# hegdepashupati/zero-inflated-gp

Hardware: AMD Instinct MI355X
Metric: elbo_steps_per_sec (higher is better)
Workload: dtype f64; 1 GPU; dense zero-inflated GP ELBO step (value+gradient), N=1000000 rows per GPU, D=3, M=1024 per latent, full batch; rows_this_rank=1000000, rows_total=1000000, M=1024, D=3, chunk_rows=32768, parallelism=row-shard x1, 1 all-reduce/step

## Files before the change

zero-inflated-gp_amd/csrc/zigp_ctx.h:

```cpp
#pragma once
#include <hip/hip_runtime.h>
#include <stdint.h>
#include <stdio.h>
#include <string.h>
#include <string>
#include <vector>
#include <map>
#include <memory>
#include "../../include/zigp.h"
#include "../../include/zigp_diag.h"
#include "zigp_gemm.h"

namespace zigp {

struct DevBuf {
  double* p = nullptr;
  size_t cap = 0;
  bool owned = true;
  DevBuf() = default;
  DevBuf(const DevBuf&) = delete;
  DevBuf& operator=(const DevBuf&) = delete;
  DevBuf(DevBuf&& o) noexcept : p(o.p), cap(o.cap), owned(o.owned) { o.p = nullptr; o.cap = 0; o.owned = true; }
  DevBuf& operator=(DevBuf&& o) noexcept {
    if (this != &o) { release(); p = o.p; cap = o.cap; owned = o.owned; o.p = nullptr; o.cap = 0; o.owned = true; }
    return *this;
  }
  ~DevBuf() { release(); }
  int ensure(size_t n) {
    if (!owned) { p = nullptr; cap = 0; owned = true; }
    if (n <= cap) return 0;
    if (p) (void)hipFree(p);
    p = nullptr; cap = 0;
    hipError_t e = hipMalloc((void**)&p, n * sizeof(double));
    if (e != hipSuccess) return -1;
    cap = n;
    return 0;
  }
  void alias(double* q, size_t n) { release(); p = q; cap = n; owned = false; }
  void release() { if (p && owned) (void)hipFree(p); p = nullptr; cap = 0; owned = true; }
};

enum ProfClass { PC_GEMM_A1 = 0, PC_GEMM_A2 = 1, PC_GEMM_H = 2, PC_GEMM_J = 3, PC_SYR2K = 4, PC_KUF = 5, PC_POINT = 6, PC_RED = 7, PC_MXM = 8, PC_OTHER = 9 };

struct TileList {
  GemmTile* d = nullptr;
  int n = 0;
  int per = 1;
};
struct HipFree { void operator()(void* q) const { (void)hipFree(q); } };
struct CachedTiles {
  std::unique_ptr<GemmTile, HipFree> d;
  int n = 0, per = 1;
  TileList view() const { return TileList{d.get(), n, per}; }
};

struct Latent {
  int M = 0, Mp = 0;
  DevBuf Z, ell, u, s, s2;
  double zc[64] = {0};
  bool kg_exact = false;
  DevBuf Zs;
  double var = 1.0;
  DevBuf Kuu, L, W;
  DevBuf K, A1, Jp;
  DevBuf Kd;
  DevBuf Wp, a1gm;
  DevBuf Wt;
  DevBuf P, Qt, Rt;
  bool P_ready = false;
  DevBuf part;
  DevBuf gm, gv;
  DevBuf du, dsq, krow;
  DevBuf xm, mom, ks0;
  DevBuf dLpart;
  DevBuf T1, T2, T3, G;
  DevBuf sk;
  DevBuf vec;
  DevBuf wh;
  DevBuf Lraw, Lq, lqssq, dLq;
};

struct KronState;
struct KfState;

struct PinnedArena {
  struct Block { char* p; size_t cap, used; };
  std::vector<Block> blocks;
  PinnedArena() = default;
  PinnedArena(const PinnedArena&) = delete;
  PinnedArena& operator=(const PinnedArena&) = delete;
  ~PinnedArena() { for (auto& b : blocks) (void)hipHostFree(b.p); }
  void reset() { for (auto& b : blocks) b.used = 0; }
  void* alloc(size_t bytes) {
    bytes = (bytes + 63) & ~(size_t)63;
    for (auto& b : blocks)
      if (b.cap - b.used >= bytes) { void* r = b.p + b.used; b.used += bytes; return r; }
    Block nb; nb.cap = bytes > ((size_t)1 << 20) ? bytes : ((size_t)1 << 20); nb.used = bytes; nb.p = nullptr;
    if (hipHostMalloc((void**)&nb.p, nb.cap, hipHostMallocDefault) != hipSuccess) return nullptr;
    blocks.push_back(nb);
    return nb.p;
  }
};

struct CtxHandles {
  hipStream_t stream = nullptr;
  hipStream_t stream_main = nullptr, stream2 = nullptr;
  hipStream_t stream3 = nullptr;
  hipEvent_t ev_fork = nullptr, ev_join = nullptr;
  hipEvent_t ev_prep_fork = nullptr, ev_prep = nullptr;
  int* d_info = nullptr;
  struct PendingEv { hipEvent_t a, b; int cls; };
  std::vector<PendingEv> pending;
  std::vector<hipEvent_t> ev_pool;
  CtxHandles() = default;
  CtxHandles(const CtxHandles&) = delete;
  CtxHandles& operator=(const CtxHandles&) = delete;
  ~CtxHandles() {
    if (d_info) (void)hipFree(d_info);
    for (auto& e : pending) { (void)hipEventDestroy(e.a); (void)hipEventDestroy(e.b); }
    for (auto e : ev_pool) (void)hipEventDestroy(e);
    for (hipEvent_t e : {ev_fork, ev_join, ev_prep_fork, ev_prep})
      if (e) (void)hipEventDestroy(e);
    for (hipStream_t s : {stream3, stream2, stream_main})
      if (s) (void)hipStreamDestroy(s);
  }
};

}

struct zigp_ctx : zigp::CtxHandles {
  ~zigp_ctx();
  int device = 0;
  std::string err;
  int info = 0;
  int64_t fit_steps_applied = 0;
  int64_t chunk = 32768;
  bool chunk_auto = true;
  const double* dX = nullptr; const double* dY = nullptr;
  zigp::DevBuf ownX, ownY;
  int64_t N = 0; int D = 0;
  const double* fullX = nullptr; const double* fullY = nullptr; int64_t fullN = 0;
  zigp::DevBuf selX, selY, selIdx;
  zigp::DevBuf fitX, fitY, fitIdx, fit;
  int64_t dense_fit_steps_applied = 0;
  zigp::Latent lat[2];
  zigp::DevBuf pw_part;
  bool fwd_kuf_side = true;
  bool trmm_tail = true;
  int overlap = 1;
  bool mean_on = false;
  bool whiten = false;
  int kern[2] = {0, 0};
  bool q_full = false;
  double mean_a[8] = {0}, mean_b = 0.0, mean_da[8] = {0}, mean_db = 0.0;
  zigp::DevBuf out9;
  zigp::DevBuf scratch, scratch2;
  zigp::PinnedArena pinned;
  std::unique_ptr<zigp::KronState> kron;
  std::unique_ptr<zigp::KfState> kronf;
  bool kron_panels = false;
  int kron_range_tiles = 1024;
  std::map<std::string, zigp::CachedTiles> tiles;
  void* comm = nullptr; int comm_rank = 0, comm_nranks = 1; int64_t comm_calls = 0;
  double comm_timeout_s = 120.0;
  zigp::DevBuf packed;
  zigp::DevBuf parm;
  double pivot_rtol = 8.0;
  bool prof_on = false;
  int prof_every = 8;
  bool prof_skip = false;
  int64_t prof_total[ZIGP_NCLASS] = {0};
  double prof_ms[ZIGP_NCLASS] = {0};
  int64_t prof_n[ZIGP_NCLASS] = {0};
  double prof_flops[ZIGP_NCLASS] = {0};
};

namespace zigp {

#define ZIGP_HIP(ctx, expr)                                                              \
  do {                                                                                   \
    hipError_t _e = (expr);                                                              \
    if (_e != hipSuccess) {                                                              \
      char _b[512];                                                                      \
      snprintf(_b, sizeof(_b), "HIP error '%s' at %s:%d (%s)", hipGetErrorString(_e), __FILE__, __LINE__, #expr); \
      (ctx)->err = _b;                                                                   \
      return ZIGP_EHIP;                                                                  \
    }                                                                                    \
  } while (0)

#define ZIGP_TRY(expr)            \
  do {                            \
    int _rc = (expr);             \
    if (_rc != 0) return _rc;     \
  } while (0)

#define ZIGP_ENSURE(ctx, buf, n)                                        \
  do {                                                                  \
    if ((buf).ensure((size_t)(n)) != 0) {                               \
      (ctx)->err = "hipMalloc failed for " #buf;                        \
      return ZIGP_EHIP;                                                 \
    }                                                                   \
  } while (0)

inline int fail_arg(zigp_ctx* c, const char* msg) { c->err = msg; return ZIGP_EARG; }
// ... 55 lines not shown
```

zero-inflated-gp_amd/csrc/zigp_dense.hip:

```cpp
#include "zigp_ctx.h"
#include "zigp_kernels.h"
#include "zigp_host.h"
#include "zigp_comm.h"
#include <algorithm>
#include <cmath>
#include <functional>

using namespace zigp;

static_assert(WIDE_MAXD == ZIGP_MAX_D, "the wide kernels' hyperparameter structs hold ZIGP_MAX_D entries");
#define ZIGP_STR2(x) #x
#define ZIGP_STR(x) ZIGP_STR2(x)
#define ZIGP_MAX_D_STR ZIGP_STR(ZIGP_MAX_D)

namespace {

enum class Param : int { Diag = 0, White = 1, WhiteFull = 2 };
constexpr bool is_white(Param p) { return p != Param::Diag; }
constexpr bool is_full(Param p) { return p == Param::WhiteFull; }
static_assert((int)Param::Diag == ZIGP_FIT_DIAG && (int)Param::White == ZIGP_FIT_WHITE && (int)Param::WhiteFull == ZIGP_FIT_WHITE_FULL,
              "Param values are the ZIGP_FIT_* modes of include/zigp.h");
Param param_of(const zigp_ctx* c) { return !c->whiten ? Param::Diag : c->q_full ? Param::WhiteFull : Param::White; }

struct HostLatent {
// ... 204 lines not shown
int latent_chunk_kuf_matern(zigp_ctx* c, Latent& lt, const double* dX, int64_t Nrows, int64_t n0, int64_t Nc, int D, const double* ell_host, int kind,
                            bool with_kd) {
  if (D < 1 || D > MAXD || !ell_host) return fail_arg(c, "a Matern Kuf panel needs 1 <= D <= 8 and host lengthscales");
  if (with_kd && lt.Kd.cap < (size_t)lt.Mp * Nc) return fail_arg(c, "a Matern gradient step's K' panel was not sized for this chunk");
  const KufHyp kh = make_kuf_hyp(ell_host, lt.var, D);
  ProfScope ps(c, PC_KUF);
  const dim3 grid((unsigned)(Nc / 512), lt.Mp / 16), block(256);
#define ZIGP_KUF_M(DD, KK, GG) \
  hipLaunchKernelGGL((k_kuf_build_matern<DD, KK, GG>), grid, block, 0, c->stream, dX, Nrows, n0, lt.Zs.p, lt.M, kh, lt.K.p, GG ? lt.Kd.p : nullptr, Nc)
#define ZIGP_KUF_MD(DD)                                                                    \
  case DD:                                                                                 \
    if (kind == ZIGP_KERN_MATERN32) { if (with_kd) ZIGP_KUF_M(DD, KERN_M32, true); else ZIGP_KUF_M(DD, KERN_M32, false); } \
    else { if (with_kd) ZIGP_KUF_M(DD, KERN_M52, true); else ZIGP_KUF_M(DD, KERN_M52, false); }                            \
    break;
  switch (D) { ZIGP_KUF_MD(1) ZIGP_KUF_MD(2) ZIGP_KUF_MD(3) ZIGP_KUF_MD(4) ZIGP_KUF_MD(5) ZIGP_KUF_MD(6) ZIGP_KUF_MD(7) ZIGP_KUF_MD(8) }
#undef ZIGP_KUF_MD
#undef ZIGP_KUF_M
  ZIGP_HIP(c, hipGetLastError());
  return 0;
}
int latent_chunk_kuf(zigp_ctx* c, Latent& lt, const double* dX, int64_t Nrows, int64_t n0, int64_t Nc, int D, const double* ell_host,
                     const double* R = nullptr, int kind = ZIGP_KERN_RBF, bool with_kd = false) {
  if (is_matern(kind)) return latent_chunk_kuf_matern(c, lt, dX, Nrows, n0, Nc, D, ell_host, kind, with_kd);
  const int Mp = lt.Mp;
  const KufHyp kh = (R || D > MAXD) ? KufHyp() : make_kuf_hyp(ell_host, lt.var, D);
  ProfScope ps(c, PC_KUF);
  const dim3 grid((unsigned)(Nc / 512), Mp / 16), block(256);
#define ZIGP_KUF(DD)                                                                                                                   \
  case DD:                                                                                                                             \
    if (R) hipLaunchKernelGGL((k_kuf_build<DD, LatHypDev>), grid, block, 0, c->stream, dX, Nrows, n0, lt.Zs.p, lt.M, LatHypDev{R, DD}, lt.K.p, Nc); \
    else hipLaunchKernelGGL((k_kuf_build<DD, KufHyp>), grid, block, 0, c->stream, dX, Nrows, n0, lt.Zs.p, lt.M, kh, lt.K.p, Nc);               \
    break;
  switch (D) {
    ZIGP_KUF(1) ZIGP_KUF(2) ZIGP_KUF(3) ZIGP_KUF(4) ZIGP_KUF(5) ZIGP_KUF(6) ZIGP_KUF(7) ZIGP_KUF(8)
    default:
      if (D < 1 || D > WIDE_MAXD || R) return fail_arg(c, "D out of range");
      hipLaunchKernelGGL(k_kuf_build_wide, grid, block, 0, c->stream, dX, Nrows, n0, lt.Zs.p, lt.M, D, make_kuf_hyp_wide(ell_host, lt.var, D), lt.K.p, Nc);
      break;
  }
#undef ZIGP_KUF
  ZIGP_HIP(c, hipGetLastError());
  return 0;
}

struct ChunkPlan {
  int64_t Nc = 0;
  bool paired = false;
  TrmmTail tail = {{0, 0}, {64, 64}};
  struct Lat { TileSpec a1_spec, a2j_spec, syr_spec, mom_spec; TileList a1, a2j, syr, mom; double fl = 0.0; } lat[2];
};
ChunkPlan chunk_plan(const int (&M)[2], int64_t Nc, Param par, bool need_grad, bool tail_on, bool wide) {
  ChunkPlan pl;
  const int nbm[2] = {ceil_div(M[0], BM), ceil_div(M[1], BM)}, nbn = (int)(Nc / BN);
  pl.Nc = Nc;
  pl.paired = trmm_paired_pays(nbn * ((nbm[0] + 1) / 2 + (nbm[1] + 1) / 2));
  if (pl.paired && tail_on)
    pl.tail = trmm_tail_plan((nbn + 7) / 8 * 8 * ((nbm[0] + 1) / 2), nbm[0], (nbn + 7) / 8 * 8 * ((nbm[1] + 1) / 2), nbm[1]);
  for (int h = 0; h < 2; ++h) {
    ChunkPlan::Lat& L = pl.lat[h];
    auto tri = [&](bool lower) { return trmm_tiles(lower, nbm[h], nbn, pl.paired, pl.tail.units[h], pl.tail.bins[h]); };
    auto full_product = [&] { return full_xcd_tiles(nbm[h], nbn, nbm[h] * (BM / BK)); };
    L.a1_spec = tri(true);
    switch (par) {
      case Param::Diag: L.a2j_spec = need_grad ? full_product() : tri(false); break;
      case Param::White: if (need_grad) L.a2j_spec = tri(false); break;
      case Param::WhiteFull: L.a2j_spec = need_grad ? full_product() : tri(false); break;
    }
    if (need_grad) L.syr_spec = syr2k_tiles(nbm[h], (int)(Nc / BK), syr_plan(nbm[h]));
    if (need_grad && wide) L.mom_spec = kgmom_tiles(nbm[h], Nc);
    L.fl = (double)M[h] * M[h] * (double)Nc;
  }
  return pl;
}
int upload_plan(zigp_ctx* c, ChunkPlan& pl) {
  for (ChunkPlan::Lat& L : pl.lat) {
    ZIGP_TRY(get_tiles(c, L.a1_spec, L.a1));
    if (L.a2j_spec.build) ZIGP_TRY(get_tiles(c, L.a2j_spec, L.a2j));
    if (L.syr_spec.build) ZIGP_TRY(get_tiles(c, L.syr_spec, L.syr));
    if (L.mom_spec.build) ZIGP_TRY(get_tiles(c, L.mom_spec, L.mom));
  }
  return 0;
}

int chunk_forward(zigp_ctx* c, const ChunkPlan& pl, Param par, bool need_grad, const std::function<int()>& after_a1 = nullptr) {
  const int64_t Nc = pl.Nc;
  struct Set { TileList t1, t2; double fl; GemmArgs a1, a2j; EpiStoreColsum e1; EpiColsum e2; EpiStorePanelKColsum ej; } q[3] = {};
  for (int h = 0; h < 2; ++h) {
    Latent& lt = c->lat[h];
    const int Mp = lt.Mp, np = Mp / 32;
    q[h].t1 = pl.lat[h].a1; q[h].t2 = pl.lat[h].a2j; q[h].fl = pl.lat[h].fl;
    q[h].a1 = mk_args(lt.Wt.p, Mp, lt.K.p, Nc, lt.A1.p, Nc);
    q[h].e1 = EpiStoreColsum{is_full(par) ? lt.wh.p + Mp : lt.vec.p, nullptr, lt.part.p, lt.part.p + (size_t)np * Nc};
    if (need_grad) {
      q[h].a2j = mk_args(lt.Rt.p, Mp, lt.A1.p, Nc, lt.Jp.p, Nc);
      q[h].ej = EpiStorePanelKColsum{lt.K.p, lt.part.p + (size_t)2 * np * Nc};
    } else {
      q[h].a2j = mk_args(is_full(par) ? lt.Lq.p : lt.W.p, Mp, lt.A1.p, Nc, nullptr, Nc);
      q[h].e2 = EpiColsum{nullptr, is_full(par) ? nullptr : lt.s2.p, nullptr, lt.part.p + (size_t)2 * np * Nc};
    }
  }
  const int groups = pl.paired ? 1 : 2;
  for (int gi = 0; gi < groups; ++gi) {
    const Set& x = q[gi];
    const Set& y = q[pl.paired ? 1 : 2];
    {
      ProfScope ps(c, PC_GEMM_A1, x.fl + y.fl);
      ZIGP_TRY((run_gemm<LAY_MNCONTIG, LAY_MNCONTIG, false, TRI_A_LOWER>(c, x.t1, x.a1, x.e1, y.t1, y.a1, y.e1)));
    }
    if (gi == groups - 1 && after_a1) ZIGP_TRY(after_a1());
    if (need_grad) {
      ProfScope ps(c, PC_GEMM_J, 2.0 * (x.fl + y.fl));
      ZIGP_TRY((run_gemm<LAY_MNCONTIG, LAY_MNCONTIG, false>(c, x.t2, x.a2j, x.ej, y.t2, y.a2j, y.ej)));
    } else {
      ProfScope ps(c, PC_GEMM_A2, x.fl + y.fl);
      ZIGP_TRY((run_gemm<LAY_MNCONTIG, LAY_MNCONTIG, false, TRI_A_UPPER>(c, x.t2, x.a2j, x.e2, y.t2, y.a2j, y.e2)));
    }
  }
  return 0;
}

int chunk_forward_white(zigp_ctx* c, const ChunkPlan& pl, bool need_grad, bool part_j, const std::function<int()>& after_a = nullptr) {
  const int64_t Nc = pl.Nc;
  struct Set { TileList t; double fl; GemmArgs g; EpiStoreColsum es; EpiColsum ec; } q[3] = {};
  for (int h = 0; h < 2; ++h) {
    Latent& lt = c->lat[h];
    const int Mp = lt.Mp, np = Mp / 32;
    double* p0 = lt.part.p; double* p2 = lt.part.p + (size_t)2 * np * Nc;
    q[h].fl = pl.lat[h].fl;
    if (part_j) { q[h].t = pl.lat[h].a2j; q[h].g = mk_args(lt.Wp.p, Mp, lt.A1.p, Nc, lt.Jp.p, Nc); continue; }
    q[h].t = pl.lat[h].a1;
    q[h].g = mk_args(lt.Wt.p, Mp, lt.K.p, Nc, need_grad ? lt.A1.p : nullptr, Nc);
    q[h].es = EpiStoreColsum{lt.wh.p + Mp, lt.wh.p, p0, p2};
    q[h].ec = EpiColsum{lt.wh.p + Mp, lt.wh.p, p0, p2};
  }
  const int groups = pl.paired ? 1 : 2;
  for (int gi = 0; gi < groups; ++gi) {
    const Set& x = q[gi];
    const Set& y = q[pl.paired ? 1 : 2];
    if (part_j) {
      ProfScope ps(c, PC_GEMM_J, x.fl + y.fl);
      ZIGP_TRY((run_gemm<LAY_MNCONTIG, LAY_MNCONTIG, false, TRI_A_UPPER>(c, x.t, x.g, EpiStore(), y.t, y.g, EpiStore())));
      continue;
    }
    {
      ProfScope ps(c, PC_GEMM_A1, x.fl + y.fl);
      if (need_grad) ZIGP_TRY((run_gemm<LAY_MNCONTIG, LAY_MNCONTIG, false, TRI_A_LOWER>(c, x.t, x.g, x.es, y.t, y.g, y.es)));
      else ZIGP_TRY((run_gemm<LAY_MNCONTIG, LAY_MNCONTIG, false, TRI_A_LOWER>(c, x.t, x.g, x.ec, y.t, y.g, y.ec)));
    }
    if (gi == groups - 1 && after_a) ZIGP_TRY(after_a());
  }
  return 0;
}

int latent_chunk_kgrad_wide(zigp_ctx* c, Latent& lt, const double* dX, int64_t Nrows, int64_t n0, int64_t Nc, int D, const TileList& mom) {
  const int Mp = lt.Mp, S = kgmom_slices(Mp / BM, Nc);
  if (mom.n != S * (Mp / BM)) return fail_arg(c, "wide Kuf gradient: the moments product's tile list was not planned for this chunk shape");
  KgCentreWide ctr;
  for (int d = 0; d < WIDE_MAXD; ++d) ctr.c[d] = lt.zc[d];
  hipLaunchKernelGGL(k_kgrad_wide_prep, dim3(Mp / KG_ROWS, KG_SPLIT), dim3(256), 0, c->stream, lt.Jp.p, lt.K.p, lt.vec.p + Mp, lt.gm.p, lt.gv.p, dX, Nrows,
                     n0, lt.M, Mp, D, Nc, (int64_t)Mp * (2 + 2 * D), ctr, lt.krow.p, lt.ks0.p, lt.xm.p);
  ZIGP_HIP(c, hipGetLastError());
  GemmArgs g = mk_args(lt.Jp.p, Nc, lt.xm.p, WIDE_MOM_COLS, lt.mom.p, WIDE_MOM_COLS);
  g.slice_stride = (int64_t)Mp * WIDE_MOM_COLS;
  ZIGP_TRY((run_gemm<LAY_KCONTIG, LAY_MNCONTIG, false>(c, mom, g, EpiStore())));
  hipLaunchKernelGGL(k_kgrad_wide_finish, dim3(Mp / 4), dim3(256), 0, c->stream, lt.mom.p, S, lt.ks0.p, lt.Z.p, lt.M, Mp, D, ctr, lt.krow.p);
  ZIGP_HIP(c, hipGetLastError());
  return 0;
}
int ensure_kgrad_wide(zigp_ctx* c, Latent& lt, int64_t Nc) {
  const int Mp = lt.Mp;
  ZIGP_ENSURE(c, lt.xm, (size_t)Nc * WIDE_MOM_COLS);
  ZIGP_ENSURE(c, lt.mom, (size_t)kgmom_slices(Mp / BM, Nc) * Mp * WIDE_MOM_COLS);
  ZIGP_ENSURE(c, lt.ks0, (size_t)KG_SPLIT * Mp);
  return 0;
}

int latent_chunk_kgrad_matern(zigp_ctx* c, Latent& lt, const double* dX, int64_t Nrows, int64_t n0, int64_t Nc, int D) {
  const int Mp = lt.Mp;
  if (D < 1 || D > MAXD) return fail_arg(c, "a Matern Kuf gradient needs 1 <= D <= 8");
  if (lt.Kd.cap < (size_t)Mp * Nc) return fail_arg(c, "a Matern gradient step's K' panel was not sized for this chunk");
  ProfScope ps(c, PC_RED);
  const dim3 gk((unsigned)ceil_div(lt.M, KG_ROWS), KG_SPLIT), bk(256);
  const int64_t slab = (int64_t)Mp * (2 + 2 * D);
#define ZIGP_KGRAD_M(DD)                                                                                                                         \
  case DD:                                                                                                                                       \
    hipLaunchKernelGGL((k_kgrad_matern<DD>), gk, bk, 0, c->stream, lt.Jp.p, lt.K.p, lt.Kd.p, lt.vec.p + Mp, lt.gm.p, lt.gv.p, dX, Nrows, n0, lt.Z.p, \
                       lt.M, Nc, slab, lt.krow.p);                                                                                               \
    break;
  switch (D) { ZIGP_KGRAD_M(1) ZIGP_KGRAD_M(2) ZIGP_KGRAD_M(3) ZIGP_KGRAD_M(4) ZIGP_KGRAD_M(5) ZIGP_KGRAD_M(6) ZIGP_KGRAD_M(7) ZIGP_KGRAD_M(8) }
#undef ZIGP_KGRAD_M
  ZIGP_HIP(c, hipGetLastError());
  return 0;
// ... 160 lines not shown
    std::string who;
    if (matern_latent(c, who))
      return fail_arg(c, ("a " + who + " (zigp_set_kernel) and D = " + std::to_string(p->D) + ": the Matern kernels cover D in [1, 8] (the wide kernels are RBF only)").c_str());
  }
  if (p->D > MAXD && c->mean_on)
    for (int d = 0; d < MAXD; ++d)
      if (c->mean_a[d] != 0.0) return fail_arg(c, "a Linear mean function is set and D > 8: Linear covers D in [1, 8] (Zero and Constant work at every D)");
  if (!p->Zf || !p->Zg || !p->u_fm || !p->u_gm || !p->u_fs_sqrt || !p->u_gs_sqrt || !p->ell_f || !p->ell_g)
    return fail_arg(c, "NULL pointer in params");
  if (!(p->var_f > 0) || !(p->var_g > 0) || !(p->noise > 0)) return fail_arg(c, "variances must be positive");
  for (int d = 0; d < p->D; ++d)
    if (!(p->ell_f[d] > 0) || !(p->ell_g[d] > 0)) return fail_arg(c, "lengthscales must be positive");
  if (c->q_full) {
    if (!c->whiten) return fail_arg(c, "zigp_set_q_full is on while whitening is off: the full-covariance q(u) exists for the whitened model only (zigp_set_whiten)");
    for (int m = 0; m < p->Mf; ++m)
      if (!(p->u_fs_sqrt[(size_t)m * p->Mf + m] != 0)) return fail_arg(c, "u_fs_sqrt has a zero (or NaN) diagonal entry (full q_sqrt, zigp_set_q_full)");
    for (int m = 0; m < p->Mg; ++m)
      if (!(p->u_gs_sqrt[(size_t)m * p->Mg + m] != 0)) return fail_arg(c, "u_gs_sqrt has a zero (or NaN) diagonal entry (full q_sqrt, zigp_set_q_full)");
    return 0;
  }
  for (int m = 0; m < p->Mf; ++m)
    if (!(p->u_fs_sqrt[m] > 0)) return fail_arg(c, "u_fs_sqrt must be positive (diagonal q_sqrt, transforms.positive)");
  for (int m = 0; m < p->Mg; ++m)
    if (!(p->u_gs_sqrt[m] > 0)) return fail_arg(c, "u_gs_sqrt must be positive (diagonal q_sqrt, transforms.positive)");
  return 0;
}

struct DenseCall {
  const zigp_params* p; const double* dX; const double* dY; int64_t Nrows; int D;
  double jitter, scale, g_offset; int64_t row_begin, row_end; int include_kl; bool predict; double* d_out9;
  bool need_grad, has_rows;
  Param par = Param::Diag;
  bool dlq_as_triangle = false;
  HostLatent hl[2]; const double* ell_h[2];
  int64_t Nc = 0;
  ChunkPlan plan[2];
  int pw_blocks = 0;
  int* hinfo = nullptr;
  bool prep_side = false;
  const double* d_hyp = nullptr; int* d_info2 = nullptr;
  const double* hyp_rec(int h) const { return d_hyp ? d_hyp + h * DH_LAT : nullptr; }
};

int dense_prepare_buffers(zigp_ctx* c, DenseCall& k);
int64_t dense_first_chunk_rows(const DenseCall& k) { return std::min<int64_t>(k.Nc, round_up(k.row_end - k.row_begin, 1024)); }
int dense_mxm_forward(zigp_ctx* c, DenseCall& k) {
  if (k.d_hyp) ZIGP_HIP(c, hipMemsetAsync(k.d_info2, 0, 2 * sizeof(int), c->stream));
  else {
    ZIGP_TRY(begin_staged_call(c));
    ZIGP_HIP(c, hipMemsetAsync(c->d_info, 0, sizeof(int), c->stream));
    ZIGP_TRY(latents_upload(c, k.hl, k.D, k.par));
  }
  k.prep_side = c->overlap == 1 && !c->prof_on;
  if (k.prep_side) {
    ZIGP_TRY(fork_side(c, c->ev_prep_fork, c->stream3));
    OnStream on(c, c->stream3);
    ZIGP_TRY(dense_prepare_buffers(c, k));
    if (k.has_rows)
      for (int h = 0; h < 2; ++h)
        ZIGP_TRY(latent_chunk_kuf(c, c->lat[h], k.dX, k.Nrows, k.row_begin, dense_first_chunk_rows(k), k.D, k.ell_h[h], k.hyp_rec(h), k.hl[h].kind,
                                  k.need_grad));
    ZIGP_HIP(c, hipEventRecord(c->ev_prep, c->stream3));
  }
  {
    ProfScope ps(c, PC_MXM);
    ZIGP_TRY(fork_side(c, c->ev_fork, c->stream2));
    ZIGP_TRY(latents_forward(c, k.hl, k.D, k.jitter, k.par, true, k.need_grad, k.d_hyp, k.d_info2));
    ZIGP_TRY(join_side(c, c->ev_join, c->stream2));
  }
  return k.d_hyp ? 0 : request_info(c, &k.hinfo);
}

int64_t auto_chunk_for(bool chunk_auto, int64_t chunk_set, int64_t Mp) {
  if (!chunk_auto) return chunk_set;
  return std::min<int64_t>(131072, std::max<int64_t>(32768, round_up(32768 * 1024 / std::max<int64_t>(Mp, 128), 1024)));
}
int64_t chunk_rows_for(bool chunk_auto, int64_t chunk_set, int64_t Mp, int64_t span) {
  int64_t chunk = auto_chunk_for(chunk_auto, chunk_set, Mp);
  if (chunk_auto && span > 0 && span <= 131072 && 4 * 2 * 8 * Mp * round_up(span, 1024) <= ((int64_t)9 << 30)) chunk = 131072;
  if (span <= 0) return 1024;
  const int64_t nchunks = (span + chunk - 1) / chunk;
  return std::max<int64_t>(1024, round_up((span + nchunks - 1) / nchunks, 1024));
}
int dense_prepare_buffers(zigp_ctx* c, DenseCall& k) {
  const int64_t Nc = k.Nc;
  const int D = k.D;
  k.pw_blocks = (int)(Nc / PW_PTS);
  ZIGP_ENSURE(c, c->pw_part, (size_t)k.pw_blocks * PW_ACC);
  ZeroRanges zr;
  zr.count = 0;
  static_assert(1 + 2 * 4 <= ZERO_RANGES_MAX, "one launch zeroes every small accumulator of a call");
  auto zero = [&](double* ptr, int64_t n) { zr.p[zr.count] = ptr; zr.n[zr.count] = n; ++zr.count; };
  zero(c->pw_part.p, (int64_t)k.pw_blocks * PW_ACC);
  for (int h = 0; h < 2; ++h) {
    Latent& lt = c->lat[h];
    const int Mp = lt.Mp;
    ZIGP_ENSURE(c, lt.gm, Nc); ZIGP_ENSURE(c, lt.gv, Nc);
    if (k.has_rows) {
      ZIGP_ENSURE(c, lt.K, (size_t)Mp * Nc);
      if (k.par != Param::White || k.need_grad) ZIGP_ENSURE(c, lt.A1, (size_t)Mp * Nc);
      ZIGP_ENSURE(c, lt.part, (size_t)3 * (Mp / 32) * Nc);
      if (k.need_grad) ZIGP_ENSURE(c, lt.Jp, (size_t)Mp * Nc);
      if (k.need_grad && is_matern(k.hl[h].kind)) ZIGP_ENSURE(c, lt.Kd, (size_t)Mp * Nc);
      if (k.need_grad && D > MAXD && !lt.kg_exact) ZIGP_TRY(ensure_kgrad_wide(c, lt, Nc));
    }
    if (k.need_grad) {
      ZIGP_ENSURE(c, lt.du, Mp); ZIGP_ENSURE(c, lt.dsq, Mp); ZIGP_ENSURE(c, lt.krow, (size_t)KG_SPLIT * Mp * (2 + 2 * D));
      const int S = syr_plan(Mp / BM).planes();
      ZIGP_ENSURE(c, lt.dLpart, (size_t)S * Mp * Mp);
      ZIGP_ENSURE(c, lt.a1gm, Mp);
      zero(lt.a1gm.p, Mp); zero(lt.du.p, Mp); zero(lt.dsq.p, Mp); zero(lt.krow.p, (int64_t)KG_SPLIT * Mp * (2 + 2 * D));
      if (k.has_rows) ZIGP_HIP(c, hipMemsetAsync(lt.dLpart.p, 0, sizeof(double) * S * Mp * Mp, c->stream));
    }
  }
  hipLaunchKernelGGL(k_zero_ranges, dim3(64), dim3(256), 0, c->stream, zr);
  ZIGP_HIP(c, hipGetLastError());
  return 0;
}

PwArgs dense_pointwise_args(zigp_ctx* c, const DenseCall& k, int64_t n0, int64_t Nc) {
  PwArgs a;
  a.part_f = c->lat[0].part.p; a.part_g = c->lat[1].part.p; a.np_f = c->lat[0].Mp / 32; a.np_g = c->lat[1].Mp / 32;
  {
    constexpr int RW2 = Shape<WavesFor<LAY_MNCONTIG, LAY_MNCONTIG, false>::value>::RW, RW1 = RW2;
    static_assert(RW1 >= 32 && RW2 >= 32, "partial-row planes are allocated for 32-row wave tiles");
    a.np1_f = c->lat[0].Mp / RW1; a.np2_f = c->lat[0].Mp / RW2; a.np1_g = c->lat[1].Mp / RW1; a.np2_g = c->lat[1].Mp / RW2;
  }
  a.Y = k.dY; a.n0 = n0; a.row_end = k.row_end; a.Nc = Nc;
  a.var_f = k.p->var_f; a.var_g = k.p->var_g; a.noise = k.p->noise; a.g_offset = k.g_offset; a.scale = k.scale;
  a.gm_f = k.need_grad ? c->lat[0].gm.p : nullptr; a.gv_f = c->lat[0].gv.p; a.gm_g = c->lat[1].gm.p; a.gv_g = c->lat[1].gv.p;
  a.X = k.dX; a.D = k.D; a.mean_on = c->mean_on ? 1 : 0; a.mean_b = c->mean_b;
  for (int d = 0; d < MAXD; ++d) a.mean_a[d] = (d < k.D) ? c->mean_a[d] : 0.0;
  a.acc = c->pw_part.p; a.out9 = k.d_out9 ? k.d_out9 - k.row_begin : nullptr; a.ld9 = k.row_end - k.row_begin;
  return a;
}
int dense_pointwise_launch(zigp_ctx* c, Param par, bool predict, bool need_grad, const PwArgs& a, const double* d_hyp) {
  ProfScope ps(c, PC_POINT);
  const dim3 grid((unsigned)(a.Nc / PW_PTS)), block(PW_THREADS);
  const bool plane2 = need_grad || d_hyp || par == Param::White;
  if (d_hyp) hipLaunchKernelGGL((k_pointwise<false, true>), grid, block, 0, c->stream, a, d_hyp);
  else if (predict && plane2) hipLaunchKernelGGL((k_pointwise<true, true>), grid, block, 0, c->stream, a);
  else if (predict) hipLaunchKernelGGL((k_pointwise<true, false>), grid, block, 0, c->stream, a);
  else if (plane2) hipLaunchKernelGGL((k_pointwise<false, true>), grid, block, 0, c->stream, a);
  else hipLaunchKernelGGL((k_pointwise<false, false>), grid, block, 0, c->stream, a);
  ZIGP_HIP(c, hipGetLastError());
  return 0;
}
int dense_pointwise(zigp_ctx* c, const DenseCall& k, int64_t n0, int64_t Nc) {
  return dense_pointwise_launch(c, k.par, k.predict, k.need_grad, dense_pointwise_args(c, k, n0, Nc), k.d_hyp);
}

int dense_chunk_loop(zigp_ctx* c, const DenseCall& k) {
  if (!k.has_rows) return 0;
  const int64_t Nc_full = k.Nc, row_begin = k.row_begin, row_end = k.row_end;
  const int D = k.D;
  auto chunk_rows = [&](int64_t n0) { return std::min<int64_t>(Nc_full, round_up(row_end - n0, 1024)); };
  auto sampled = [&](int64_t n0) {
    if (!c->prof_on) return false;
    if (c->prof_every <= 1 || row_end - row_begin <= Nc_full) return true;
    return chunk_rows(n0) == Nc_full && (((n0 - row_begin) / Nc_full) % c->prof_every) == 0;
  };
  auto kuf = [&](int64_t n0) -> int {
    for (int h = 0; h < 2; ++h)
      ZIGP_TRY(latent_chunk_kuf(c, c->lat[h], k.dX, k.Nrows, n0, chunk_rows(n0), D, k.ell_h[h], k.hyp_rec(h), k.hl[h].kind, k.need_grad));
    return 0;
  };
  auto kgrad = [&](int64_t n0, int64_t Nc) -> int {
    const ChunkPlan& pl = k.plan[Nc == k.plan[0].Nc ? 0 : 1];
    for (int h = 0; h < 2; ++h) ZIGP_TRY(latent_chunk_kgrad(c, c->lat[h], k.dX, k.Nrows, n0, Nc, D, k.ell_h[h], pl.lat[h].mom, k.hl[h].kind));
    return 0;
  };
  bool side_busy = false;
  auto on_side = [&](auto work) -> int {
    ZIGP_TRY(fork_side(c, c->ev_fork, c->stream2));
    OnStream on(c, c->stream2);
    ZIGP_TRY(work());
    ZIGP_HIP(c, hipEventRecord(c->ev_join, c->stream2));
    side_busy = true;
    return 0;
  };
  auto wait_side = [&]() -> int {
    if (side_busy) ZIGP_HIP(c, hipStreamWaitEvent(c->stream_main, c->ev_join, 0));
    side_busy = false;
    return 0;
  };
  c->prof_skip = c->prof_on && !sampled(row_begin);
  if (!k.prep_side) ZIGP_TRY(kuf(row_begin));
  for (int64_t n0 = row_begin; n0 < row_end; n0 += Nc_full) {
    const int64_t Nc = chunk_rows(n0);
    const int64_t n1 = n0 + Nc_full;
    const bool has_next = n1 < row_end;
    const bool timed = sampled(n0), timed_next = has_next && sampled(n1);
    c->prof_skip = c->prof_on && !timed;
    ZIGP_TRY(wait_side());
    const bool kuf_fwd_side = c->overlap == 1 && c->fwd_kuf_side && !k.need_grad && has_next && !timed && !timed_next;
    std::function<int()> after_a1;
    if (kuf_fwd_side) after_a1 = [&] { return on_side([&] { return kuf(n1); }); };
    const ChunkPlan& pl = k.plan[Nc == k.plan[0].Nc ? 0 : 1];
    if (k.par == Param::White) {
      ZIGP_TRY(chunk_forward_white(c, pl, k.need_grad, false, after_a1));
      ZIGP_TRY(dense_pointwise(c, k, n0, Nc));
      if (k.need_grad) ZIGP_TRY(chunk_forward_white(c, pl, true, true));
    } else {
      ZIGP_TRY(chunk_forward(c, pl, k.par, k.need_grad, after_a1));
      ZIGP_TRY(dense_pointwise(c, k, n0, Nc));
    }
    const bool kgrad_side = c->overlap == 1 && k.need_grad && !timed;
    const bool kuf_side = kgrad_side && has_next && !timed_next;
    if (kgrad_side)
      ZIGP_TRY(on_side([&]() -> int {
        ZIGP_TRY(kgrad(n0, Nc));
        return kuf_side ? kuf(n1) : 0;
      }));
    if (k.need_grad) {
      if (!kgrad_side) ZIGP_TRY(kgrad(n0, Nc));
      for (int h = 0; h < 2; ++h) ZIGP_TRY(latent_chunk_syrk(c, pl, h));
    }
    if (has_next && !kuf_side && !kuf_fwd_side) {
      ZIGP_TRY(wait_side());
      c->prof_skip = c->prof_on && !timed_next;
      ZIGP_TRY(kuf(n1));
    }
  }
  return wait_side();
}

int dense_pack(zigp_ctx* c, const DenseCall& k, DensePackArgs& a, size_t& n) {
  const int D = k.D;
  n = DP_HDR;
  memset(&a, 0, sizeof(a));
  for (int h = 0; h < 2; ++h) {
    Latent& lt = c->lat[h];
    DensePackLat& L = a.lat[h];
    L.krow = lt.krow.p; L.du = lt.du.p; L.dsq = lt.dsq.p; L.vec = lt.vec.p; L.s = lt.s.p; L.ell = lt.ell.p;
    if (is_white(k.par)) { L.du = lt.a1gm.p; L.vec = lt.wh.p; }
    L.M = lt.M; L.Mp = lt.Mp; L.var = lt.var; L.out_off = (int64_t)n; L.q_full = is_full(k.par) ? 1 : 0;
    L.ns = !is_full(k.par) ? (int64_t)lt.M : k.dlq_as_triangle ? (int64_t)lt.M * (lt.M + 1) / 2 : (int64_t)lt.M * lt.M;
    if (k.need_grad) n += (size_t)lt.M * D + (size_t)lt.M + (size_t)L.ns + D;
  }
  a.pw = c->pw_part.p; a.pw_blocks = k.pw_blocks; a.D = D; a.need_grad = k.need_grad ? 1 : 0; a.include_kl = k.include_kl ? 1 : 0;
  a.mean_on = c->mean_on ? 1 : 0;
  ZIGP_ENSURE(c, c->packed, n);
  a.out = c->packed.p;
  if (k.d_hyp) hipLaunchKernelGGL(k_dense_pack<const double*>, dim3(2), dim3(256), 0, c->stream, a, k.d_hyp);
  else hipLaunchKernelGGL(k_dense_pack<>, dim3(2), dim3(256), 0, c->stream, a);
  if (k.need_grad && is_full(k.par))
    for (int h = 0; h < 2; ++h) {
      const Latent& lt = c->lat[h];
      double* os = a.out + a.lat[h].out_off + (int64_t)lt.M * D + lt.M;
      const dim3 grid(ceil_div((int64_t)lt.M * lt.M, 256));
      if (k.dlq_as_triangle) hipLaunchKernelGGL(k_pack_tril, grid, dim3(256), 0, c->stream, lt.dLq.p, lt.M, (int64_t)lt.Mp, os);
      else hipLaunchKernelGGL(k_pack_square, grid, dim3(256), 0, c->stream, lt.dLq.p, lt.M, (int64_t)lt.Mp, os);
    }
  ZIGP_HIP(c, hipGetLastError());
  return 0;
}
int dense_gather(zigp_ctx* c, DenseCall& k, double* elbo_data, double* kl, zigp_grads* grads) {
  const int D = k.D;
  size_t n = 0;
  DensePackArgs a;
  ZIGP_TRY(dense_pack(c, k, a, n));
  ZIGP_TRY(comm_allreduce(c, c->packed.p, n));
  double* hv = nullptr;
  ZIGP_TRY(download(c, c->packed.p, n, &hv));
  ZIGP_HIP(c, hipStreamSynchronize(c->stream));
  prof_collect(c);
  ZIGP_TRY(info_result(c, k.hinfo, "Kuu"));
  if (elbo_data) *elbo_data = hv[0];
  if (kl) *kl = hv[1];
  c->mean_db = hv[5];
// ... 8 lines not shown
      const double* o = hv + a.lat[h].out_off;
      if (gZ[h]) memcpy(gZ[h], o, sizeof(double) * M * D);
      if (gu[h]) memcpy(gu[h], o + M * D, sizeof(double) * M);
      const size_t ns = is_full(k.par) ? M * M : M;
      if (gs[h]) memcpy(gs[h], o + M * D + M, sizeof(double) * ns);
      if (gl[h]) memcpy(gl[h], o + M * D + M + ns, sizeof(double) * D);
    }
    grads->var_f = hv[2]; grads->var_g = hv[3]; grads->noise = hv[4];
  }
  return 0;
}

int dense_plan(zigp_ctx* c, DenseCall& k) {
  const int M[2] = {k.hl[0].M, k.hl[1].M};
  const int64_t span = k.has_rows ? k.row_end - k.row_begin : 0;
  k.Nc = chunk_rows_for(c->chunk_auto, c->chunk, round_up(std::max(M[0], M[1]), BM), span);
  if (k.has_rows) {
    const int64_t last = std::min<int64_t>(k.Nc, round_up(span - (span - 1) / k.Nc * k.Nc, 1024));
    k.plan[0] = chunk_plan(M, k.Nc, k.par, k.need_grad, c->trmm_tail, k.D > MAXD);
    ZIGP_TRY(upload_plan(c, k.plan[0]));
    if (last != k.Nc) { k.plan[1] = chunk_plan(M, last, k.par, k.need_grad, c->trmm_tail, k.D > MAXD); ZIGP_TRY(upload_plan(c, k.plan[1])); }
  }
  return 0;
}
int dense_step(zigp_ctx* c, DenseCall& k) {
  ZIGP_TRY(dense_mxm_forward(c, k));
  if (k.prep_side) ZIGP_HIP(c, hipStreamWaitEvent(c->stream_main, c->ev_prep, 0));
  else ZIGP_TRY(dense_prepare_buffers(c, k));
  const int rc = dense_chunk_loop(c, k);
  c->prof_skip = false;
  ZIGP_TRY(rc);
  if (k.need_grad) {
    ProfScope ps(c, PC_MXM);
    ZIGP_TRY(fork_side(c, c->ev_fork, c->stream2));
    for (int h = 0; h < 2; ++h) {
      OnStream on(c, h == 0 ? c->stream_main : c->stream2);
      ZIGP_TRY(latent_mxm_backward(c, c->lat[h], k.D, k.jitter, k.par, k.has_rows, k.include_kl != 0, nullptr, &k.hl[h]));
    }
    ZIGP_TRY(join_side(c, c->ev_join, c->stream2));
  }
  return 0;
}

int run_dense(zigp_ctx* c, const zigp_params* p, const double* dX, const double* dY, int64_t Nrows, int D, double jitter,
              double scale, double g_offset, int64_t row_begin, int64_t row_end, int include_kl, bool predict, double* d_out9,
              double* elbo_data, double* kl, zigp_grads* grads) {
  DenseCall k;
  k.p = p; k.dX = dX; k.dY = dY; k.Nrows = Nrows; k.D = D; k.jitter = jitter; k.scale = scale; k.g_offset = g_offset;
  k.row_begin = row_begin; k.row_end = row_end; k.include_kl = include_kl; k.predict = predict; k.d_out9 = d_out9;
  k.need_grad = (grads != nullptr) && !predict;
  k.has_rows = row_end > row_begin;
  k.par = param_of(c);
  k.hl[0] = HostLatent{p->Mf, p->Zf, p->u_fm, p->u_fs_sqrt, p->ell_f, p->var_f, c->kern[0]};
  k.hl[1] = HostLatent{p->Mg, p->Zg, p->u_gm, p->u_gs_sqrt, p->ell_g, p->var_g, c->kern[1]};
  k.ell_h[0] = p->ell_f; k.ell_h[1] = p->ell_g;
  ZIGP_TRY(dense_plan(c, k));
  ZIGP_TRY(dense_step(c, k));
  if (predict) { ZIGP_HIP(c, hipStreamSynchronize(c->stream)); prof_collect(c); return info_result(c, k.hinfo, "Kuu"); }
  return dense_gather(c, k, elbo_data, kl, grads);
}

}

extern "C" {

int zigp_create(zigp_ctx** out, int device_id) {
  if (!out) return ZIGP_EARG;
  *out = nullptr;
  int ndev = 0;
  if (hipGetDeviceCount(&ndev) != hipSuccess || ndev <= 0) return ZIGP_EHIP;
  if (device_id < 0 || device_id >= ndev) return ZIGP_EARG;
  if (hipSetDevice(device_id) != hipSuccess) return ZIGP_EHIP;
  zigp_ctx* c = new (std::nothrow) zigp_ctx();
  if (!c) return ZIGP_EHIP;
  c->device = device_id;
  if (hipStreamCreateWithFlags(&c->stream, hipStreamNonBlocking) != hipSuccess) { delete c; return ZIGP_EHIP; }
  c->stream_main = c->stream;
  if (hipStreamCreateWithFlags(&c->stream2, hipStreamNonBlocking) != hipSuccess) { delete c; return ZIGP_EHIP; }
  if (hipStreamCreateWithFlags(&c->stream3, hipStreamNonBlocking) != hipSuccess) { delete c; return ZIGP_EHIP; }
  if (hipEventCreateWithFlags(&c->ev_fork, hipEventDisableTiming) != hipSuccess ||
      hipEventCreateWithFlags(&c->ev_join, hipEventDisableTiming) != hipSuccess ||
      hipEventCreateWithFlags(&c->ev_prep_fork, hipEventDisableTiming) != hipSuccess ||
      hipEventCreateWithFlags(&c->ev_prep, hipEventDisableTiming) != hipSuccess) { delete c; return ZIGP_EHIP; }
  if (hipMalloc((void**)&c->d_info, sizeof(int)) != hipSuccess) { delete c; return ZIGP_EHIP; }
  if (hipFuncSetAttribute(reinterpret_cast<const void*>(&k_potrf_diag<double>), hipFuncAttributeMaxDynamicSharedMemorySize,
                          (int)(sizeof(double) * PB * PBLD)) != hipSuccess ||
      hipFuncSetAttribute(reinterpret_cast<const void*>(&k_potrf_diag<const double*>), hipFuncAttributeMaxDynamicSharedMemorySize,
                          (int)(sizeof(double) * PB * PBLD)) != hipSuccess) { delete c; return ZIGP_EHIP; }
  if (const char* e = getenv("ZIGP_FWD_KUF_SIDE")) c->fwd_kuf_side = atoi(e) != 0;
  if (const char* e = getenv("ZIGP_TRMM_TAIL")) c->trmm_tail = atoi(e) != 0;
  if (const char* e = getenv("ZIGP_COMM_TIMEOUT_S")) { const double v = atof(e); if (v > 0) c->comm_timeout_s = v; }
  *out = c;
  return ZIGP_OK;
}

int zigp_destroy(zigp_ctx* c) {
  if (!c) return ZIGP_EARG;
  (void)hipSetDevice(c->device);
  (void)hipStreamSynchronize(c->stream_main);
  (void)hipStreamSynchronize(c->stream2);
  if (c->stream3) (void)hipStreamSynchronize(c->stream3);
  if (c->comm) { RcclApi* api = rccl_api(nullptr); if (api) (void)api->CommDestroy(static_cast<ncclComm_t>(c->comm)); c->comm = nullptr; }
  delete c;
  return ZIGP_OK;
}

const char* zigp_last_error(zigp_ctx* c) { return c ? c->err.c_str() : "null context"; }
int zigp_last_info(zigp_ctx* c) { return c ? c->info : 0; }

int zigp_set_overlap(zigp_ctx* c, int32_t on) {
  if (!c) return ZIGP_EARG;
  if (on < 0 || on > 1) return fail_arg(c, "zigp_set_overlap: mode must be 0 or 1");
  c->overlap = on;
  return ZIGP_OK;
}

int zigp_set_chunk(zigp_ctx* c, int64_t chunk_rows) {
  if (!c) return ZIGP_EARG;
  if (chunk_rows == 0) { c->chunk_auto = true; c->chunk = 32768; return ZIGP_OK; }
  if (chunk_rows < 1024 || chunk_rows % 1024 != 0) return fail_arg(c, "chunk must be a positive multiple of 1024 (or 0: automatic)");
  if (chunk_rows > (1 << 20)) return fail_arg(c, "chunk must be <= 1048576 rows (32-bit staging offsets; 3 panels (K, A1, J') of 8*M*chunk bytes per latent)");
  c->chunk = chunk_rows;
  c->chunk_auto = false;
  return ZIGP_OK;
}

int zigp_set_pivot_rtol(zigp_ctx* c, double rtol) {
  if (!c) return ZIGP_EARG;
  if (!(rtol >= 0) || !std::isfinite(rtol)) return fail_arg(c, "zigp_set_pivot_rtol: rtol must be finite and >= 0");
  c->pivot_rtol = rtol;
  return ZIGP_OK;
}

int64_t zigp_get_chunk(zigp_ctx* c, int32_t M) {
  if (!c || M <= 0) return ZIGP_EARG;
  return auto_chunk_for(c->chunk_auto, c->chunk, round_up(M, BM));
}

int64_t zigp_get_chunk_rows(zigp_ctx* c, int32_t M, int64_t span) {
  if (!c || M <= 0 || span < 0) return ZIGP_EARG;
  return chunk_rows_for(c->chunk_auto, c->chunk, round_up(M, BM), span);
}

static_assert(MAXD == 8, "zigp_ctx::mean_a / mean_da hold MAXD entries");

int zigp_set_mean_function(zigp_ctx* c, const double* a, int32_t D, double b) {
  if (!c) return ZIGP_EARG;
  if (D < -1 || D > MAXD || (D > 0 && !a)) return fail_arg(c, "zigp_set_mean_function: need -1 <= D <= 8 and a[D] (a Linear mean function covers D in [1, 8]; Zero and Constant work at every D)");
  if (D < 0) {
    for (int d = 0; d < MAXD; ++d) c->mean_a[d] = 0.0;
    c->mean_b = 0.0; c->mean_on = false;
    return ZIGP_OK;
  }
  if (!std::isfinite(b)) return fail_arg(c, "zigp_set_mean_function: b must be finite");
  for (int d = 0; d < D; ++d)
    if (!std::isfinite(a[d])) return fail_arg(c, "zigp_set_mean_function: a must be finite");
  for (int d = 0; d < MAXD; ++d) c->mean_a[d] = (d < D) ? a[d] : 0.0;
  c->mean_b = b;
  c->mean_on = true;
  return ZIGP_OK;
}

int zigp_set_whiten(zigp_ctx* c, int32_t on) {
  if (!c) return ZIGP_EARG;
  if (on < 0 || on > 1) return fail_arg(c, "zigp_set_whiten: on must be 0 or 1");
  c->whiten = on != 0;
// ... 1160 lines not shown
```

Before: 7.403 ELBO steps/s (value+gradient, 1e6-row steps, fp64).

## Software-pipeline dense chunk loop with double-buffered Kuf/A1 across streams

```diff
diff --git a/zero-inflated-gp_amd/csrc/zigp_ctx.h b/zero-inflated-gp_amd/csrc/zigp_ctx.h
--- a/zero-inflated-gp_amd/csrc/zigp_ctx.h
+++ b/zero-inflated-gp_amd/csrc/zigp_ctx.h
@@ -63,6 +63,8 @@
   double var = 1.0;
   DevBuf Kuu, L, W;
   DevBuf K, A1, Jp;
+  DevBuf K_alt, A1_alt, part_alt;
+  int slot = 0;
   DevBuf Kd;
   DevBuf Wp, a1gm;
   DevBuf Wt;
@@ -108,6 +110,7 @@
   hipStream_t stream3 = nullptr;
   hipEvent_t ev_fork = nullptr, ev_join = nullptr;
   hipEvent_t ev_prep_fork = nullptr, ev_prep = nullptr;
+  hipEvent_t ev_kuf[2] = {nullptr, nullptr};
   int* d_info = nullptr;
   struct PendingEv { hipEvent_t a, b; int cls; };
   std::vector<PendingEv> pending;
@@ -119,7 +122,7 @@
     if (d_info) (void)hipFree(d_info);
     for (auto& e : pending) { (void)hipEventDestroy(e.a); (void)hipEventDestroy(e.b); }
     for (auto e : ev_pool) (void)hipEventDestroy(e);
-    for (hipEvent_t e : {ev_fork, ev_join, ev_prep_fork, ev_prep})
+    for (hipEvent_t e : {ev_fork, ev_join, ev_prep_fork, ev_prep, ev_kuf[0], ev_kuf[1]})
       if (e) (void)hipEventDestroy(e);
     for (hipStream_t s : {stream3, stream2, stream_main})
       if (s) (void)hipStreamDestroy(s);
diff --git a/zero-inflated-gp_amd/csrc/zigp_dense.hip b/zero-inflated-gp_amd/csrc/zigp_dense.hip
--- a/zero-inflated-gp_amd/csrc/zigp_dense.hip
+++ b/zero-inflated-gp_amd/csrc/zigp_dense.hip
@@ -310,7 +310,9 @@
   return 0;
 }
 
-int chunk_forward(zigp_ctx* c, const ChunkPlan& pl, Param par, bool need_grad, const std::function<int()>& after_a1 = nullptr) {
+enum ChunkForwardPart { CF_BOTH, CF_A1, CF_SECOND };
+int chunk_forward(zigp_ctx* c, const ChunkPlan& pl, Param par, bool need_grad, const std::function<int()>& after_a1 = nullptr,
+                  ChunkForwardPart part = CF_BOTH) {
   const int64_t Nc = pl.Nc;
   struct Set { TileList t1, t2; double fl; GemmArgs a1, a2j; EpiStoreColsum e1; EpiColsum e2; EpiStorePanelKColsum ej; } q[3] = {};
   for (int h = 0; h < 2; ++h) {
@@ -331,11 +333,12 @@
   for (int gi = 0; gi < groups; ++gi) {
     const Set& x = q[gi];
     const Set& y = q[pl.paired ? 1 : 2];
-    {
+    if (part != CF_SECOND) {
       ProfScope ps(c, PC_GEMM_A1, x.fl + y.fl);
       ZIGP_TRY((run_gemm<LAY_MNCONTIG, LAY_MNCONTIG, false, TRI_A_LOWER>(c, x.t1, x.a1, x.e1, y.t1, y.a1, y.e1)));
     }
     if (gi == groups - 1 && after_a1) ZIGP_TRY(after_a1());
+    if (part == CF_A1) continue;
     if (need_grad) {
       ProfScope ps(c, PC_GEMM_J, 2.0 * (x.fl + y.fl));
       ZIGP_TRY((run_gemm<LAY_MNCONTIG, LAY_MNCONTIG, false>(c, x.t2, x.a2j, x.ej, y.t2, y.a2j, y.ej)));
@@ -662,6 +665,19 @@
   const int64_t nchunks = (span + chunk - 1) / chunk;
   return std::max<int64_t>(1024, round_up((span + nchunks - 1) / nchunks, 1024));
 }
+#ifndef ZIGP_CHUNK_PIPE
+#define ZIGP_CHUNK_PIPE 1
+#endif
+bool chunk_pipe_applies(const zigp_ctx* c, const DenseCall& k) {
+  if (!ZIGP_CHUNK_PIPE) return false;
+  return k.has_rows && k.need_grad && c->overlap == 1 && !c->prof_on && k.row_end - k.row_begin > k.Nc && k.par != Param::White && k.D <= MAXD &&
+         !is_matern(k.hl[0].kind) && !is_matern(k.hl[1].kind);
+}
+void latent_use_slot(Latent& lt, int s) {
+  if (lt.slot == s) return;
+  std::swap(lt.K, lt.K_alt); std::swap(lt.A1, lt.A1_alt); std::swap(lt.part, lt.part_alt);
+  lt.slot = s;
+}
 int dense_prepare_buffers(zigp_ctx* c, DenseCall& k) {
   const int64_t Nc = k.Nc;
   const int D = k.D;
@@ -681,6 +697,9 @@
       if (k.par != Param::White || k.need_grad) ZIGP_ENSURE(c, lt.A1, (size_t)Mp * Nc);
       ZIGP_ENSURE(c, lt.part, (size_t)3 * (Mp / 32) * Nc);
       if (k.need_grad) ZIGP_ENSURE(c, lt.Jp, (size_t)Mp * Nc);
+      if (chunk_pipe_applies(c, k)) {
+        ZIGP_ENSURE(c, lt.K_alt, (size_t)Mp * Nc); ZIGP_ENSURE(c, lt.A1_alt, (size_t)Mp * Nc); ZIGP_ENSURE(c, lt.part_alt, (size_t)3 * (Mp / 32) * Nc);
+      }
       if (k.need_grad && is_matern(k.hl[h].kind)) ZIGP_ENSURE(c, lt.Kd, (size_t)Mp * Nc);
       if (k.need_grad && D > MAXD && !lt.kg_exact) ZIGP_TRY(ensure_kgrad_wide(c, lt, Nc));
     }
@@ -766,6 +785,49 @@
   };
   c->prof_skip = c->prof_on && !sampled(row_begin);
   if (!k.prep_side) ZIGP_TRY(kuf(row_begin));
+  if (chunk_pipe_applies(c, k)) {
+    struct Slot0 { zigp_ctx* c; ~Slot0() { for (Latent& lt : c->lat) latent_use_slot(lt, 0); } } back_to_slot0{c};
+    auto use_slot = [&](int64_t i) { for (Latent& lt : c->lat) latent_use_slot(lt, (int)(i % 2)); };
+    auto plan_of = [&](int64_t Nc) -> const ChunkPlan& { return k.plan[Nc == k.plan[0].Nc ? 0 : 1]; };
+    auto row0 = [&](int64_t i) { return row_begin + i * Nc_full; };
+    const int64_t nchunks = (row_end - row_begin + Nc_full - 1) / Nc_full;
+    {
+      ZIGP_TRY(fork_side(c, c->ev_fork, c->stream2));
+      OnStream on(c, c->stream2);
+      use_slot(1);
+      ZIGP_TRY(kuf(row0(1)));
+      ZIGP_HIP(c, hipEventRecord(c->ev_kuf[1], c->stream2));
+    }
+    use_slot(0);
+    ZIGP_TRY(chunk_forward(c, plan_of(chunk_rows(row0(0))), k.par, true, nullptr, CF_A1));
+    for (int64_t i = 0; i < nchunks; ++i) {
+      const int64_t n0 = row0(i), Nc = chunk_rows(n0);
+      const ChunkPlan& pl = plan_of(Nc);
+      use_slot(i);
+      ZIGP_TRY(wait_side());
+      ZIGP_TRY(chunk_forward(c, pl, k.par, true, nullptr, CF_SECOND));
+      ZIGP_TRY(dense_pointwise(c, k, n0, Nc));
+      if (i + 1 < nchunks) {
+        ZIGP_HIP(c, hipStreamWaitEvent(c->stream_main, c->ev_kuf[(i + 1) % 2], 0));
+        use_slot(i + 1);
+        ZIGP_TRY(chunk_forward(c, plan_of(chunk_rows(row0(i + 1))), k.par, true, nullptr, CF_A1));
+        use_slot(i);
+      }
+      {
+        ZIGP_TRY(fork_side(c, c->ev_fork, c->stream2));
+        OnStream on(c, c->stream2);
+        ZIGP_TRY(kgrad(n0, Nc));
+        ZIGP_HIP(c, hipEventRecord(c->ev_join, c->stream2));
+        side_busy = true;
+        if (i + 2 < nchunks) {
+          ZIGP_TRY(kuf(row0(i + 2)));
+          ZIGP_HIP(c, hipEventRecord(c->ev_kuf[i % 2], c->stream2));
+        }
+      }
+      for (int h = 0; h < 2; ++h) ZIGP_TRY(latent_chunk_syrk(c, pl, h));
+    }
+    return wait_side();
+  }
   for (int64_t n0 = row_begin; n0 < row_end; n0 += Nc_full) {
     const int64_t Nc = chunk_rows(n0);
     const int64_t n1 = n0 + Nc_full;
@@ -940,6 +1002,8 @@
       hipEventCreateWithFlags(&c->ev_join, hipEventDisableTiming) != hipSuccess ||
       hipEventCreateWithFlags(&c->ev_prep_fork, hipEventDisableTiming) != hipSuccess ||
       hipEventCreateWithFlags(&c->ev_prep, hipEventDisableTiming) != hipSuccess) { delete c; return ZIGP_EHIP; }
+  for (hipEvent_t* e : {&c->ev_kuf[0], &c->ev_kuf[1]})
+    if (hipEventCreateWithFlags(e, hipEventDisableTiming) != hipSuccess) { delete c; return ZIGP_EHIP; }
   if (hipMalloc((void**)&c->d_info, sizeof(int)) != hipSuccess) { delete c; return ZIGP_EHIP; }
   if (hipFuncSetAttribute(reinterpret_cast<const void*>(&k_potrf_diag<double>), hipFuncAttributeMaxDynamicSharedMemorySize,
                           (int)(sizeof(double) * PB * PBLD)) != hipSuccess ||
```

New measurement: 7.421 ELBO steps/s (value+gradient, 1e6-row steps, fp64), median of 6. No clear change (+0.2%).
